# EloDoyard/movie-recommender-system

Hardware: AMD Instinct MI355X
Metric: test-set predictions/sec (kNN k=300, fit+predict+MAE) (higher is better)
Workload: dtype fp16 MFMA similarity filter (fp32 acc) + f64 exact re-rank/prediction

## Files before the change

### movie-recommender-system_amd/csrc/api.cpp

```cpp
#include <math.h>
#include <stdio.h>
#include <string.h>

#include <algorithm>
#include <vector>

#include "engine.h"

using namespace knncf;

namespace knncf {
void launch_first_rows(int64_t n, const int32_t* d_du, const int32_t* d_di, int32_t own_lo, int32_t own_hi,
                       uint32_t* d_first, hipStream_t st);
void launch_length_keys(int32_t count, const int32_t* d_list, const int64_t* d_u_ptr, int32_t max_len, uint64_t* d_key, hipStream_t st);
void launch_collect_new(int32_t U, const uint32_t* d_first, int64_t* d_seq, int64_t epoch, int32_t own_lo, int32_t own_hi,
                        int32_t* d_list, int32_t* d_count, hipStream_t st);
void launch_fallback_keys(int32_t U, const double* d_exact, uint64_t* d_keys, uint32_t* d_vals, hipStream_t st);
void launch_fallback_write(int32_t user, int32_t take, int32_t kcap, const uint32_t* d_sorted_vals,
                           const double* d_exact, int32_t* nbr_idx, double* nbr_sim, int32_t* nbr_cnt,
                           hipStream_t st);
void launch_jaccard_pair(const Train& tr, int32_t u, int32_t v, double* d_out, hipStream_t st);
}

struct StageTimer {
// ... 24 lines not shown
    DArr<bf16_t> Apanel[2];
    DArr<float> S[2];
    DArr<float> S_full;
    DArr<uint32_t> sym_tiles;
    DArr<int32_t> redo_rows;
    int32_t sym_tiles_n = 0;
    hipEvent_t ev_produced[2] = {nullptr, nullptr}, ev_consumed[2] = {nullptr, nullptr}, ev_ready = nullptr;
    int32_t* pinned_cnt = nullptr;
    size_t pinned_cap = 0;
    SelectScratch sel;
    SliceScratch slices;
    NeighborTable pt;
    bool pt_ready = false;
    PersonalRows prow;
    bool prow_ready = false;
    DArr<int32_t> reco_users, reco_items, reco_out_items;
    DArr<double> reco_pred, reco_out_preds;
    DArr<uint8_t> reco_rated;
    QueryScratch query;
    QueryBatchScratch query_batch;
    DArr<int32_t> build_list, build_count;
    DArr<uint32_t> first_row;
    DArr<int32_t> t_du, t_di, t_users, t_items;
    DArr<double> t_pred, t_err, t_ratings, t_partial, scalar_out;
    DArr<unsigned long long> scalar_u64;
    DArr<uint8_t> t_owned;
    DArr<int64_t> t_counts;
    DArr<int32_t> sweep_ks;
    std::vector<uint32_t> h_ukeys, h_ikeys;
    std::vector<int32_t> h_uid;
    knncf_timings tm{};
    std::vector<StageTimer> pending;
    std::vector<hipEvent_t> event_pool;
};

namespace {

hipEvent_t get_event(knncf_handle* h) {
    if (!h->event_pool.empty()) {
        hipEvent_t e = h->event_pool.back();
        h->event_pool.pop_back();
        return e;
    }
    hipEvent_t e;
    KN_HIP(hipEventCreate(&e));
    return e;
// ... 30 lines not shown
template <class F>
int guarded(knncf_handle* h, F&& f) {
    if (!h) return KNNCF_E_INVALID;
    struct DeviceGuard {
        int prev = -1;
        ~DeviceGuard() { if (prev >= 0) (void)hipSetDevice(prev); }
    } guard;
    try {
        int cur = -1;
        if (hipGetDevice(&cur) != hipSuccess) {
            (void)hipGetLastError();
            KN_HIP(hipSetDevice(h->cfg.device));
        } else if (cur != h->cfg.device) {
            guard.prev = cur;
            KN_HIP(hipSetDevice(h->cfg.device));
        }
        f();
        resolve_timers(h);
        return KNNCF_OK;
    } catch (const Error& e) {
        h->err = e.what();
        (void)hipStreamSynchronize(h->stream);
        (void)hipStreamSynchronize(h->stream2);
        (void)hipGetLastError();
        h->pending.clear();
        return e.status;
    } catch (const std::bad_alloc&) {
        h->err = "host allocation failed";
        return KNNCF_E_NOMEM;
    } catch (const std::exception& e) {
        h->err = e.what();
        return KNNCF_E_INVALID;
    }
}

void require_fitted(knncf_handle* h, bool committed = true) {
    KN_REQUIRE(h->fitted, KNNCF_E_STATE, "call knncf_fit first");
    if (committed) KN_REQUIRE(h->committed, KNNCF_E_STATE, "sharded handle: call knncf_shard_commit after the exchange");
}

void load_host_ids(knncf_handle* h) {
    if (!h->h_ukeys.empty() || h->tr.U == 0) return;
    Train& tr = h->tr;
    h->h_ukeys.resize(tr.U);
    h->h_ikeys.resize(tr.I);
    h->h_uid.resize(tr.U);
// ... 86 lines not shown
        const double frac = (double)rows_total / (double)tr.U;
        const double U_pad = (double)round_up(tr.U, 256);
        double best = 1e300;
        H = I;
        for (int64_t cand = 64;; cand += 64) {
            int32_t hc = (int32_t)std::min<int64_t>(cand, I);
            double cost = 2.0 * rows_total * U_pad * (double)round_up(hc, 64) / RATE_DENSE + tail_sq[hc] * frac / RATE_SPARSE;
            if (cost < best) { best = cost; H = hc; }
            if (hc == I) break;
        }
        if (tr.jaccard && (h->cfg.flags & KNNCF_FLAG_F32_PANEL) == 0) H = std::min(H, 2048);
    }
    h->tail_pairs_full = tail_sq[H];
    return H;
}

void build_neighbors(knncf_handle* h, int32_t count) {
    Train& tr = h->tr;
    NeighborTable& nt = h->nt;
    if (count <= 0 || nt.kcap <= 0) return;
    KN_REQUIRE(h->cfg.similarity != KNNCF_SIM_ONE, KNNCF_E_UNSUPPORTED,
               "kNN neighbourhoods with similarityOne: every similarity is 1.0, the neighbourhood is the first k users in Set order — not built");
    hipStream_t st = h->stream;
    if (count > 256) {
        PrepScratch& sc = h->prep;
        sc.k64_a.ensure(count); sc.k64_b.ensure(count); sc.v32_b.ensure(count);
        launch_length_keys(count, h->build_list.p, tr.u_ptr.p, tr.I, sc.k64_a.p, st);
        sort_pairs_u64_u32(sc.sort, sc.k64_a.p, sc.k64_b.p, reinterpret_cast<const uint32_t*>(h->build_list.p), sc.v32_b.p, count, bits_for((uint64_t)tr.I), st);
        KN_HIP(hipMemcpyAsync(h->build_list.p, sc.v32_b.p, (size_t)count * sizeof(int32_t), hipMemcpyDeviceToDevice, st));
    }
    const bool fp16 = (h->cfg.flags & KNNCF_FLAG_BF16_FILTER) == 0;
    const bool s_fp16 = (h->cfg.flags & KNNCF_FLAG_F32_PANEL) == 0;
    h->U_pad = round_up(tr.U, 256);
    const int64_t U_pad = h->U_pad;
    size_t free_b = 0, total_b = 0;
    KN_HIP(hipMemGetInfo(&free_b, &total_b));
    const int64_t s_elem = s_fp16 ? 2 : 4;
    const size_t sym_bytes = (size_t)U_pad * (size_t)U_pad * (size_t)s_elem;
    size_t own = h->S_full.bytes() + h->sel.cand_idx.bytes() + h->sel.cand_approx.bytes() + h->sel.grp_v0.bytes() + h->sel.grp_x.bytes();
    for (int s = 0; s < 2; ++s) own += h->S[s].bytes() + h->Apanel[s].bytes();
    bool use_sym = h->cfg.shard_count == 1 && (int64_t)count * 2 >= tr.U && U_pad / 256 < 65536 &&
                   sym_bytes <= (free_b + own) / 3 && !getenv("KNNCF_DEBUG_NO_SYMMETRIC_GEMM");
    if (use_sym) {
        try {
            h->S_full.ensure((sym_bytes + 3) / 4);
        } catch (const Error& e) {
            if (e.status != KNNCF_E_NOMEM) throw;
            (void)hipGetLastError();
            use_sym = false;
        }
    }
    if (!h->b_ready) {
        h->head = choose_head(h, count, use_sym);
        h->K_pad = round_up(h->head, 64);
        size_t need = (size_t)U_pad * h->K_pad * sizeof(bf16_t);
        KN_REQUIRE(need < free_b + h->Bpanel.bytes(), KNNCF_E_UNSUPPORTED,
                   "dense bf16 user panel does not fit in HBM; lower head_items");
        Stage s(h, &h->tm.densify_ms);
        h->colmap.ensure(tr.I);
        launch_colmap(tr, h->head, h->colmap.p, st);
        h->Bpanel.ensure((size_t)U_pad * h->K_pad);
        launch_densify(tr, nullptr, 0, tr.U, h->colmap.p, h->Bpanel.p, h->K_pad, U_pad, fp16, st);
        if (tr.jaccard) {
            KN_REQUIRE(!s_fp16 || h->head <= 2048, KNNCF_E_UNSUPPORTED, "Jaccard: more than 2048 dense head items need KNNCF_FLAG_F32_PANEL");
            h->row_len.ensure((size_t)row_len_size(tr.U));
            launch_row_len(tr, h->row_len.p, st);
        }
        if (h->head < tr.I) {
            h->te_cnt.ensure(tr.U); h->te_item.ensure(tr.n); h->te_x.ensure(tr.n);
            h->row_tail_abs.ensure(tr.U); h->row_head_sq.ensure(tr.U);
            launch_tail_entries(tr, h->colmap.p, h->te_cnt.p, h->te_item.p, h->te_x.p, h->row_tail_abs.p, h->row_head_sq.p, st);
        }
        h->b_ready = true;
        KN_HIP(hipMemGetInfo(&free_b, &total_b));
    }
    const int64_t K_pad = h->K_pad;
    const int32_t head = h->head;
    h->tm.head_items = head;
    if (use_sym) {
        const int32_t n_tiles = (int32_t)(U_pad / 256);
        if (h->sym_tiles_n != n_tiles) {
            std::vector<uint32_t> list;
            gemm_sym_tile_list(n_tiles, list);
            h->sym_tiles.ensure(list.size());
            KN_HIP(hipMemcpyAsync(h->sym_tiles.p, list.data(), list.size() * sizeof(uint32_t), hipMemcpyHostToDevice, st));
            KN_HIP(hipStreamSynchronize(st));
            h->sym_tiles_n = n_tiles;
        }
        const int64_t n_listed = (int64_t)n_tiles * (n_tiles + 1) / 2;
        Stage s(h, &h->tm.gemm_ms);
        launch_gemm_sym(h->Bpanel.p, h->S_full.p, s_fp16, U_pad, h->K_pad, h->K_pad, U_pad, fp16, !tr.jaccard, h->sym_tiles.p, n_listed, st);
        h->tm.gemm_launches += 1;
        h->tm.gemm_flops_executed += 2.0 * 256.0 * 256.0 * (double)n_listed * (double)h->K_pad;
        h->tm.gemm_flops_algorithmic += 2.0 * (double)count * (double)(tr.U - 1) * (double)h->head;
        KN_HIP(hipMemGetInfo(&free_b, &total_b));
// ... 85 lines not shown
    };
    const bool per_block_redo = !use_sym && n_blocks > 1;
    for (int64_t b = 0; b < n_blocks; ++b) {
        const int64_t rb = b * R;
        const int32_t rows = (int32_t)std::min<int64_t>(R, count - rb);
        const int64_t M = round_up(rows, 256);
        const int32_t* d_rows = h->build_list.p + rb;
        const int slot = (int)(b % slots);
        if (b >= slots) KN_HIP(hipStreamWaitEvent(sp, h->ev_consumed[slot], 0));
        if (!use_sym) {
            Stage s(h, &h->tm.densify_ms, sp);
            launch_densify(tr, d_rows, 0, rows, h->colmap.p, h->Apanel[slot].p, K_pad, M, fp16, sp);
        }
        if (!use_sym) {
            Stage s(h, &h->tm.gemm_ms, sp);
            launch_gemm_nt(h->Apanel[slot].p, h->Bpanel.p, h->S[slot].p, s_fp16, M, U_pad, K_pad, K_pad, K_pad, U_pad, fp16, !tr.jaccard, sp);
            h->tm.gemm_launches += 1;
            h->tm.gemm_flops_executed += 2.0 * (double)M * (double)U_pad * (double)K_pad;
            h->tm.gemm_flops_algorithmic += 2.0 * (double)rows * (double)(tr.U - 1) * (double)head;
        }
        KN_HIP(hipEventRecord(h->ev_produced[slot], sp));
        KN_HIP(hipStreamWaitEvent(sc, h->ev_produced[slot], 0));
        TailEntries te{h->te_cnt.p, h->te_item.p, h->te_x.p, h->row_tail_abs.p, h->row_head_sq.p, h->row_len.p};
        h->prep.join_commit(sc);
        const void* Sblk = use_sym ? (const void*)h->S_full.p : (const void*)h->S[slot].p;
        const int32_t gcap = select_gcap(nt.k);
        auto select_rows = [&](int32_t r0, int32_t nr) {
            Stage s(h, &h->tm.select_ms, sc);
            const void* Sp = use_sym ? Sblk : (const void*)(static_cast<const char*>(Sblk) + (size_t)r0 * (size_t)U_pad * (size_t)s_elem);
            launch_tail_select(tr, h->colmap.p, te, head < tr.I, Sp, use_sym, s_fp16, U_pad, nr, d_rows + r0, nt.k, eps_opnd, eps_rest, cap,
                               h->sel.cand_idx.p + (size_t)r0 * cap, h->sel.cand_approx.p + (size_t)r0 * cap, h->sel.cand_cnt.p + r0, h->sel.cand_eps.p + r0,
                               h->sel.grp_v0.p + (size_t)r0 * gcap, h->sel.grp_x.p + (size_t)r0 * gcap * 8, gcap, sc);
            h->tm.select_launches += 1;
            h->tm.tail_pair_updates += h->tail_pairs_full * ((double)nr / (double)tr.U);
            h->tm.select_row_bytes += (double)s_elem * (double)nr * (double)tr.U;
        };
        const int32_t slices = std::min<int32_t>(8, 8192 / std::max<int32_t>(nt.kcap, 1));
        const char* force_slices = getenv("KNNCF_DEBUG_SLICE_ROWS");
        const int32_t n_heavy = slices < 2                         ? 0
                                : force_slices                     ? std::max<int32_t>(0, std::min<int32_t>(rows, atoi(force_slices)))
                                : (rows >= 4096 && rows <= 65536)  ? std::max<int32_t>(16, rows / 512)
                                                                   : 0;
        select_rows(0, rows);
        if (overlap && !per_block_redo) KN_HIP(hipEventRecord(h->ev_consumed[slot], sc));
        {
            Stage s(h, &h->tm.rerank_ms, sc);
// ... 175 lines not shown
        KN_HIP(hipStreamSynchronize(st));
    }
    const int64_t n_blocks = std::max<int64_t>(1, ceil_div(nu, R));
    for (int64_t b = 0; b < n_blocks; ++b) {
        const int64_t u0 = b * R, u1 = std::min<int64_t>(nu, u0 + R);
        const int64_t r0 = b == 0 ? 0 : first_row[u0], r1 = b + 1 < n_blocks ? first_row[u1] : n;
        if (u1 > u0) {
            Stage s(h, &h->tm.rerank_ms);
            launch_sim_rows(tr, pr, pr.users.p + u0, (int32_t)(u1 - u0), pr.S.p, st);
        }
        Stage s(h, &h->tm.predict_ms);
        launch_fold_rows(tr, pr, r1 - r0, sc.v32_b.p + r0, h->t_du.p, h->t_di.p, d_ratings, pr.slot.p, pr.S.p, d_pred, h->t_err.p,
                         h->t_owned.p, st);
    }
}

void ensure_item_stats(knncf_handle* h) {
    if (h->tr.item_stats_ready) return;
    Stage s(h, &h->tm.prep_ms);
    h->prep.join_commit(h->stream);
    prep_item_stats(h->tr, h->prep, h->stream);
}

int64_t order_test_rows(knncf_handle* h, int64_t n, bool by_item, int32_t cols) {
    Train& tr = h->tr;
    hipStream_t st = h->stream;
    PrepScratch& sc = h->prep;
    sc.k64_a.ensure(n); sc.k64_b.ensure(n); sc.v32_a.ensure(n); sc.v32_b.ensure(n);
    const uint32_t key_limit = (uint32_t)(by_item ? tr.I : tr.U);
    if (h->cfg.shard_count > 1) {
        h->scalar_u64.ensure(1);
        KN_HIP(hipMemsetAsync(h->scalar_u64.p, 0, sizeof(unsigned long long), st));
        KN_HIP(hipMemsetAsync(h->t_err.p, 0, (size_t)cols * (size_t)n * sizeof(double), st));
        KN_HIP(hipMemsetAsync(h->t_owned.p, 0, (size_t)n, st));
        launch_owned_keys(n, by_item ? h->t_di.p : h->t_du.p, h->t_du.p, tr.own_lo, tr.own_hi, h->cfg.shard_rank == 0, key_limit,
                          sc.k64_a.p, sc.v32_a.p, h->scalar_u64.p, st);
        sort_pairs_u64_u32(sc.sort, sc.k64_a.p, sc.k64_b.p, sc.v32_a.p, sc.v32_b.p, n, bits_for((uint64_t)key_limit + 1), st);
        return (int64_t)fetch(h, h->scalar_u64.p, 0);
    }
    launch_user_keys(n, by_item ? h->t_di.p : h->t_du.p, key_limit, sc.k64_a.p, sc.v32_a.p, st);
    sort_pairs_u64_u32(sc.sort, sc.k64_a.p, sc.k64_b.p, sc.v32_a.p, sc.v32_b.p, n, bits_for((uint64_t)key_limit), st);
    return n;
}

void reduce_errors(knncf_handle* h, int64_t n, int32_t cols, double* sums, int64_t* count) {
    hipStream_t st = h->stream;
    const int32_t nb = 1024;
    h->t_partial.ensure((size_t)nb * cols);
    h->t_counts.ensure((size_t)nb * cols);
    for (int32_t c = 0; c < cols; ++c)
        launch_reduce_err(h->t_err.p + (size_t)c * n, h->t_owned.p, n, h->t_partial.p + (size_t)c * nb, h->t_counts.p + (size_t)c * nb, nb, st);
    std::vector<double> hp((size_t)nb * cols);
    std::vector<int64_t> hc((size_t)nb * cols);
    KN_HIP(hipMemcpyAsync(hp.data(), h->t_partial.p, hp.size() * sizeof(double), hipMemcpyDeviceToHost, st));
    KN_HIP(hipMemcpyAsync(hc.data(), h->t_counts.p, hc.size() * sizeof(int64_t), hipMemcpyDeviceToHost, st));
    KN_HIP(hipStreamSynchronize(st));
    for (int32_t c = 0; c < cols; ++c) {
        double s_ = 0.0;
        int64_t c_ = 0;
        for (int32_t b = 0; b < nb; ++b) { s_ += hp[(size_t)c * nb + b]; c_ += hc[(size_t)c * nb + b]; }
        if (sums) sums[c] = s_;
        if (count && c == 0) *count = c_;
    }
}

// ... 9 lines not shown
    KN_REQUIRE(d_users && d_items, KNNCF_E_INVALID, "null test arrays");
    int kind = predictor;
    NeighborTable* table = &h->nt;
    bool stream = false;
    if (predictor == KNNCF_PRED_PERSONALIZED) {
        if (h->cfg.similarity == KNNCF_SIM_ONE) {
            kind = KNNCF_PRED_BASELINE_RDD;
        } else if (personalized_streams(h)) {
            ensure_personal_rows(h);
            stream = true;
        } else {
            ensure_personalized_table(h);
            kind = KNNCF_PRED_KNN;
            table = &h->pt;
        }
    }
    KN_REQUIRE(stream || (kind >= KNNCF_PRED_GLOBAL_AVG && kind <= KNNCF_PRED_KNN), KNNCF_E_INVALID, "unknown predictor");
    if (kind == KNNCF_PRED_ITEM_AVG || kind == KNNCF_PRED_BASELINE || kind == KNNCF_PRED_BASELINE_RDD) ensure_item_stats(h);
    ensure_test_scratch(h, n);
    {
        Stage s(h, &h->tm.predict_ms);
        launch_dense_ids(tr, d_users, d_items, n, h->t_du.p, h->t_di.p, st);
    }
    if (kind == KNNCF_PRED_KNN && table == &h->nt) ensure_neighbors_for_rows(h, n);
    h->prep.join_commit(st);
    double* pred = d_pred_out ? d_pred_out : h->t_pred.p;
    if (stream) predict_personal_rows(h, d_ratings, n, pred);
    {
        Stage s(h, &h->tm.predict_ms);
        const uint32_t* d_order = nullptr;
        const bool by_item = tr.ib_words > 0 && tr.ib_words * 12 <= 48 * 1024;
        int64_t n_rows = n;
        if (kind == KNNCF_PRED_KNN) {
            n_rows = order_test_rows(h, n, by_item, 1);
            d_order = h->prep.v32_b.p;
        }
        if (n_rows > 0 && !stream)
            launch_predict(tr, table, kind, n_rows, h->t_du.p, h->t_di.p, d_ratings, d_order, by_item, pred, h->t_err.p, h->t_owned.p,
                           h->cfg.shard_rank == 0, st);
        if (sum_abs_err || count) reduce_errors(h, n, 1, sum_abs_err, count);
    }
}

void check_sweep_ks(const int32_t* ks, int32_t n_k) {
    KN_REQUIRE(ks && n_k >= 1 && n_k <= 64, KNNCF_E_INVALID, "sweep: 1 .. 64 values of k");
    for (int32_t q = 0; q < n_k; ++q)
        KN_REQUIRE(ks[q] >= 1 && ks[q] <= 2048 && (q == 0 || ks[q] > ks[q - 1]), KNNCF_E_INVALID,
                   "sweep: k must be strictly ascending in [1, 2048]");
}

void run_mae_sweep(knncf_handle* h, const int32_t* ks, int32_t n_k, const int32_t* d_users, const int32_t* d_items,
                   const double* d_ratings, int64_t n, double* sums, int64_t* count, double* d_pred) {
    check_sweep_ks(ks, n_k);
    require_fitted(h);
    KN_REQUIRE(h->cfg.similarity != KNNCF_SIM_ONE, KNNCF_E_UNSUPPORTED,
               "kNN neighbourhoods with similarityOne: every similarity is 1.0, the neighbourhood is the first k users in Set order — not built");
    KN_REQUIRE(n >= 0, KNNCF_E_INVALID, "negative row count");
    for (int32_t q = 0; q < n_k; ++q) sums[q] = 0.0;
    *count = 0;
    if (n == 0) return;
    KN_REQUIRE(d_users && d_items && d_ratings, KNNCF_E_INVALID, "null test arrays");
    Train& tr = h->tr;
    hipStream_t st = h->stream;
    struct Restore {
        knncf_handle* h;
        int32_t k;
        ~Restore() {
            h->cfg.k = k;
            try { reset_neighbors(h); } catch (const Error&) {}
        }
    } restore{h, h->cfg.k};
    h->cfg.k = ks[n_k - 1];
    reset_neighbors(h);
    ensure_test_scratch(h, n);
    h->t_err.ensure((size_t)n_k * n);
    {
        Stage s(h, &h->tm.predict_ms);
        launch_dense_ids(tr, d_users, d_items, n, h->t_du.p, h->t_di.p, st);
    }
    ensure_neighbors_for_rows(h, n);
    h->prep.join_commit(st);
    std::vector<int32_t> hk(ks, ks + n_k);
    h->sweep_ks.ensure(64);
    KN_HIP(hipMemcpyAsync(h->sweep_ks.p, hk.data(), (size_t)n_k * sizeof(int32_t), hipMemcpyHostToDevice, st));
    {
        Stage s(h, &h->tm.predict_ms);
        const int64_t n_rows = order_test_rows(h, n, true, n_k);
        if (n_rows > 0)
            launch_predict_sweep(tr, h->nt, h->sweep_ks.p, n_k, n_rows, n, h->t_du.p, h->t_di.p, d_ratings, h->prep.v32_b.p, d_pred,
                                 h->t_err.p, h->t_owned.p, h->cfg.shard_rank == 0, st);
        reduce_errors(h, n, n_k, sums, count);
    }
}

void do_fit_device(knncf_handle* h, const int32_t* d_users, const int32_t* d_items, const double* d_ratings, int64_t n) {
    KN_REQUIRE(n > 0 && d_users && d_items && d_ratings, KNNCF_E_INVALID, "fit: null or empty input");
    Train& tr = h->tr;
    hipStream_t st = h->stream;
    h->fitted = h->committed = false;
    h->short_rows = -1;
    h->b_ready = false;
    h->pt_ready = false;
    h->prow_ready = false;
    h->h_ukeys.clear(); h->h_ikeys.clear(); h->h_uid.clear();
    tr.n = n;
    tr.jaccard = h->cfg.similarity == KNNCF_SIM_JACCARD;
    {
        Stage s(h, &h->tm.prep_ms);
        if (tr.user_raw.p != d_users) {
            tr.user_raw.alloc(n); tr.item_raw.alloc(n); tr.rating.alloc(n);
            KN_HIP(hipMemcpyAsync(tr.user_raw.p, d_users, n * sizeof(int32_t), hipMemcpyDeviceToDevice, st));
            KN_HIP(hipMemcpyAsync(tr.item_raw.p, d_items, n * sizeof(int32_t), hipMemcpyDeviceToDevice, st));
// ... 401 lines not shown
}

int knncf_create(const knncf_config* cfg, knncf_handle** out) {
    if (!cfg || !out || cfg->struct_size != sizeof(knncf_config)) return KNNCF_E_INVALID;
    if (cfg->shard_count < 1 || cfg->shard_rank < 0 || cfg->shard_rank >= cfg->shard_count || cfg->k < 0)
        return KNNCF_E_INVALID;
    if (cfg->similarity < KNNCF_SIM_COSINE || cfg->similarity > KNNCF_SIM_JACCARD) return KNNCF_E_INVALID;
    int ndev = 0;
    if (hipGetDeviceCount(&ndev) != hipSuccess || ndev <= 0 || cfg->device < 0 || cfg->device >= ndev) {
        (void)hipGetLastError();
        return KNNCF_E_NODEVICE;
    }
    hipDeviceProp_t prop;
    if (hipGetDeviceProperties(&prop, cfg->device) != hipSuccess) return KNNCF_E_NODEVICE;
    if (strncmp(prop.gcnArchName, "gfx950", 6) != 0) return KNNCF_E_NODEVICE;
    knncf_handle* h = new (std::nothrow) knncf_handle();
    if (!h) return KNNCF_E_NOMEM;
    h->cfg = *cfg;
    if (hipSetDevice(cfg->device) != hipSuccess || hipStreamCreateWithFlags(&h->stream, hipStreamNonBlocking) != hipSuccess ||
        hipStreamCreateWithFlags(&h->stream2, hipStreamNonBlocking) != hipSuccess) {
        delete h;
        return KNNCF_E_HIP;
    }
    bool ok = hipEventCreateWithFlags(&h->ev_ready, hipEventDisableTiming) == hipSuccess;
    for (int s = 0; s < 2; ++s) {
        ok = ok && hipEventCreateWithFlags(&h->ev_produced[s], hipEventDisableTiming) == hipSuccess;
        ok = ok && hipEventCreateWithFlags(&h->ev_consumed[s], hipEventDisableTiming) == hipSuccess;
    }
    if (!ok) {
        knncf_destroy(h);
        return KNNCF_E_HIP;
    }
    *out = h;
    return KNNCF_OK;
}

void knncf_destroy(knncf_handle* h) {
    if (!h) return;
    (void)hipSetDevice(h->cfg.device);
    (void)hipStreamSynchronize(h->stream);
    for (auto& t : h->pending) { (void)hipEventDestroy(t.a); (void)hipEventDestroy(t.b); }
    for (auto e : h->event_pool) (void)hipEventDestroy(e);
    if (h->stream2) (void)hipStreamSynchronize(h->stream2);
    if (h->ev_ready) (void)hipEventDestroy(h->ev_ready);
    for (int s = 0; s < 2; ++s) {
        if (h->ev_produced[s]) (void)hipEventDestroy(h->ev_produced[s]);
// ... 446 lines not shown
```

### movie-recommender-system_amd/csrc/engine.h

```cpp
#pragma once

#include <string>
#include <vector>

#include "common.h"

namespace knncf {

typedef __bf16 bf16_t;

inline int32_t select_gcap(int32_t k) { return 8192 * (int32_t)((k + 511) / 512 > 1 ? (k + 511) / 512 : 1); }
static constexpr int SELECT_TCOLS = 16384;
static_assert(SELECT_TCOLS <= 16384 && (SELECT_TCOLS & (SELECT_TCOLS - 1)) == 0, "it_pack: 16-bit cell byte address");

struct SortWorkspace {
    DArr<char> tmp;
    DArr<size_t> count;
};
void sort_pairs_u64_u32(SortWorkspace& ws, const uint64_t* kin, uint64_t* kout, const uint32_t* vin,
                        uint32_t* vout, size_t n, int end_bit, hipStream_t st);
void sort_keys_u32(SortWorkspace& ws, const uint32_t* kin, uint32_t* kout, size_t n, hipStream_t st);
void sort_pairs_u32_u32(SortWorkspace& ws, const uint32_t* kin, uint32_t* kout, const uint32_t* vin, uint32_t* vout, size_t n,
                        int end_bit, hipStream_t st);
size_t unique_u32(SortWorkspace& ws, const uint32_t* sorted_in, uint32_t* out, size_t n, hipStream_t st);
// ... 36 lines not shown
    int64_t own_p0 = 0, own_p1 = 0;
    bool jaccard = false;
};

enum : uint32_t { ST_NONFINITE = 1u, ST_DUPLICATE = 2u, ST_NOT_DYADIC = 4u, ST_LONG_ROW = 16u };

struct PrepScratch {
    SortWorkspace sort;
    DArr<uint64_t> k64_a, k64_b;
    DArr<uint32_t> v32_a, v32_b, k32_a, k32_b;
    DArr<int32_t> du_row, di_row;
    DArr<uint32_t> perm_f;
    DArr<uint32_t> status;
    DArr<int32_t> idrange;
    DArr<uint32_t> ucnt, utile;
    DArr<int32_t> long_rows;
    DArr<double> dsum;
    DArr<uint4> rec;
    hipStream_t aux = nullptr;
    hipEvent_t ev_fork = nullptr, ev_join = nullptr, ev_commit = nullptr;
    bool commit_pending = false;
    DArr<uint32_t> perm_iu;
    void join_commit(hipStream_t st);
    void ensure_aux();
    void release_all();
    PrepScratch() = default;
    PrepScratch(const PrepScratch&) = delete;
    PrepScratch& operator=(const PrepScratch&) = delete;
    ~PrepScratch();
};

void prep_fit(Train& tr, PrepScratch& sc, int32_t shard_rank, int32_t shard_count, hipStream_t st);
void prep_complete_rows(Train& tr, PrepScratch& sc, hipStream_t st);
void prep_commit(Train& tr, PrepScratch& sc, hipStream_t st);
void prep_item_stats(Train& tr, PrepScratch& sc, hipStream_t st);

void launch_dense_ids(const Train& tr, const int32_t* d_users, const int32_t* d_items, int64_t n,
                      int32_t* d_du, int32_t* d_di, hipStream_t st);

void launch_densify(const Train& tr, const int32_t* d_rows, int32_t row_begin, int32_t n_rows,
                    const int32_t* d_colmap, bf16_t* panel, int64_t ld, int64_t panel_rows, bool fp16,
                    hipStream_t st);
void launch_colmap(const Train& tr, int32_t H, int32_t* d_colmap, hipStream_t st);
void launch_gemm_nt(const bf16_t* A, const bf16_t* B, void* C, bool c_fp16, int64_t M, int64_t N, int64_t K,
                    int64_t lda, int64_t ldb, int64_t ldc, bool fp16, bool clamp, hipStream_t st);

// ... 180 lines not shown
```

### movie-recommender-system_amd/csrc/prep.hip

```cpp
#include <math.h>

#include <algorithm>
#include <vector>

#include <stdlib.h>

#include "engine.h"

namespace knncf {

static constexpr int TPB = 256;
static inline int nblocks(int64_t n, int per = TPB) { return (int)std::max<int64_t>(1, ceil_div(n, per)); }

void PrepScratch::ensure_aux() {
    if (aux) return;
    KN_HIP(hipStreamCreateWithFlags(&aux, hipStreamNonBlocking));
    KN_HIP(hipEventCreateWithFlags(&ev_fork, hipEventDisableTiming));
    KN_HIP(hipEventCreateWithFlags(&ev_join, hipEventDisableTiming));
    KN_HIP(hipEventCreateWithFlags(&ev_commit, hipEventDisableTiming));
}
void PrepScratch::join_commit(hipStream_t st) {
    if (!commit_pending) return;
    KN_HIP(hipStreamWaitEvent(st, ev_commit, 0));
    commit_pending = false;
}
PrepScratch::~PrepScratch() {
    if (aux) { (void)hipStreamSynchronize(aux); (void)hipStreamDestroy(aux); }
    if (ev_fork) (void)hipEventDestroy(ev_fork);
    if (ev_join) (void)hipEventDestroy(ev_join);
    if (ev_commit) (void)hipEventDestroy(ev_commit);
}

void PrepScratch::release_all() {
    sort.tmp.release();
    k64_a.release(); k64_b.release(); v32_a.release(); v32_b.release();
    k32_a.release(); k32_b.release(); du_row.release(); di_row.release(); perm_f.release(); rec.release(); long_rows.release(); ucnt.release(); utile.release(); perm_iu.release();
}

__global__ void k_row_keys(int64_t n, const int32_t* __restrict__ users, const int32_t* __restrict__ items,
                           uint32_t* __restrict__ ukey, uint32_t* __restrict__ ikey) {
    int64_t t = (int64_t)blockIdx.x * blockDim.x + threadIdx.x;
    if (t >= n) return;
    ukey[t] = int_trie_key(users[t]);
    ikey[t] = int_trie_key(items[t]);
}

__global__ void __launch_bounds__(TPB) k_id_range(int64_t n, const int32_t* __restrict__ users, const int32_t* __restrict__ items,
                                                  int32_t* __restrict__ idrange) {
    __shared__ int32_t part[4][TPB / 64];
    int32_t u = 0x7fffffff, i = 0x7fffffff, um = (int32_t)0x80000000, im = (int32_t)0x80000000;
    for (int64_t t = (int64_t)blockIdx.x * TPB + threadIdx.x; t < n; t += (int64_t)gridDim.x * TPB) {
        const int32_t a = users[t], b = items[t];
        u = min(u, a); um = max(um, a);
        i = min(i, b); im = max(im, b);
    }
#pragma unroll
    for (int o = 32; o > 0; o >>= 1) {
// ... 542 lines not shown
}

template <bool SQUARE>
static void fold(const int64_t* seg_ptr, int32_t lo, int32_t hi, const uint32_t* perm, const double* src,
                 double* out, hipStream_t st, int32_t spb = TPB) {
    if (hi <= lo) return;
    k_ordered_fold<SQUARE><<<nblocks(hi - lo, spb), TPB, 0, st>>>(seg_ptr, lo, hi, spb, perm, src, out);
    KN_HIP(hipGetLastError());
}

static uint32_t read_status(PrepScratch& sc, hipStream_t st) {
    uint32_t h = 0;
    KN_HIP(hipMemcpyAsync(&h, sc.status.p, sizeof(uint32_t), hipMemcpyDeviceToHost, st));
    KN_HIP(hipStreamSynchronize(st));
    return h;
}

void prep_fit(Train& tr, PrepScratch& sc, int32_t shard_rank, int32_t shard_count, hipStream_t st) {
    const int64_t n = tr.n;
    KN_REQUIRE(n > 0, KNNCF_E_INVALID, "fit: empty training set");
    KN_REQUIRE(n < (int64_t)1 << 29, KNNCF_E_UNSUPPORTED, "fit: more than 2^29-1 ratings (the kernels address the rating arrays with 32-bit byte offsets)");
    if (sc.aux) KN_HIP(hipStreamSynchronize(sc.aux));
    sc.commit_pending = false;
    sc.status.ensure(4);
    KN_HIP(hipMemsetAsync(sc.status.p, 0, 4 * sizeof(uint32_t), st));
    sc.k32_a.ensure(n); sc.k32_b.ensure(n); sc.v32_a.ensure(n); sc.v32_b.ensure(n);
    sc.k64_a.ensure(n); sc.k64_b.ensure(n);

    uint32_t* ukey_row = sc.k32_a.p;
    uint32_t* ikey_row = sc.v32_a.p;
    bool have_row_keys = false;
    sc.idrange.ensure(4);
    {
        const int32_t init[4] = {0x7fffffff, (int32_t)0x80000000, 0x7fffffff, (int32_t)0x80000000};
        KN_HIP(hipMemcpyAsync(sc.idrange.p, init, sizeof(init), hipMemcpyHostToDevice, st));
    }
    k_id_range<<<(unsigned)std::min<int64_t>(1024, ceil_div(n, TPB)), TPB, 0, st>>>(n, tr.user_raw.p, tr.item_raw.p, sc.idrange.p);
    k_check_dyadic<<<nblocks(n), TPB, 0, st>>>(n, tr.rating.p, sc.status.p);
    KN_HIP(hipGetLastError());
    int32_t rg[4];
    uint32_t early_status = 0;
    KN_HIP(hipMemcpyAsync(rg, sc.idrange.p, sizeof(rg), hipMemcpyDeviceToHost, st));
    KN_HIP(hipMemcpyAsync(&early_status, sc.status.p, sizeof(uint32_t), hipMemcpyDeviceToHost, st));
    KN_HIP(hipStreamSynchronize(st));
    const bool dyadic = !(early_status & ST_NOT_DYADIC);
    const int32_t ID_LIMIT = 1 << 24;
    const bool small_ids = rg[0] >= 0 && rg[2] >= 0 && rg[1] < ID_LIMIT && rg[3] < ID_LIMIT && !getenv("KNNCF_DEBUG_NO_ID_TABLES");
    tr.u_table_n = tr.i_table_n = 0;
    size_t U = 0, I = 0;
    if (small_ids) {
        tr.u_table_n = rg[1] + 1;
        tr.i_table_n = rg[3] + 1;
        tr.u_table.ensure(tr.u_table_n);
        tr.i_table.ensure(tr.i_table_n);
        KN_HIP(hipMemsetAsync(tr.u_table.p, 0xff, (size_t)tr.u_table_n * sizeof(int32_t), st));
        KN_HIP(hipMemsetAsync(tr.i_table.p, 0xff, (size_t)tr.i_table_n * sizeof(int32_t), st));
        k_mark_ids<<<nblocks(n), TPB, 0, st>>>(n, tr.user_raw.p, tr.item_raw.p, tr.u_table.p, tr.i_table.p);
        KN_HIP(hipMemsetAsync(sc.status.p + 2, 0, 2 * sizeof(uint32_t), st));
        k_table_keys<<<nblocks(tr.u_table_n), TPB, 0, st>>>(tr.u_table_n, tr.u_table.p, sc.k32_b.p, sc.status.p + 2);
        k_table_keys<<<nblocks(tr.i_table_n), TPB, 0, st>>>(tr.i_table_n, tr.i_table.p, sc.v32_b.p, sc.status.p + 3);
        KN_HIP(hipGetLastError());
        uint32_t cnt[2];
        KN_HIP(hipMemcpyAsync(cnt, sc.status.p + 2, sizeof(cnt), hipMemcpyDeviceToHost, st));
        KN_HIP(hipStreamSynchronize(st));
        U = cnt[0];
        I = cnt[1];
// ... 155 lines not shown
        if (n > 4) {
            k_make_keys<<<nblocks(n), TPB, 0, st>>>(n, 2, sc.du_row.p, sc.di_row.p, tr.user_raw.p, tr.item_raw.p, sc.k64_a.p, 32);
            sort_pairs_u64_u32(sc.sort, sc.k64_a.p, sc.k64_b.p, sc.perm_f.p, tr.perm_uh.p, n, 32 + ubits, st);
        }
    } else if (!seg_sorts && p1 > p0) {
        const int tbits = bits_for((uint64_t)n);
        k_slice_file_keys<<<nblocks(p1 - p0), TPB, 0, st>>>(p0, p1 - p0, lo, tr.s_user.p, tr.s_t.p, tbits, sc.k64_a.p, sc.v32_a.p);
        KN_HIP(hipGetLastError());
        sort_pairs_u64_u32(sc.sort, sc.k64_a.p, sc.k64_b.p, sc.v32_a.p, tr.perm_uf.p + p0, p1 - p0, tbits + bits_for((uint64_t)(hi - lo)), st);
        if (n > 4) {
            k_slice_hash_keys<<<nblocks(p1 - p0), TPB, 0, st>>>(p1 - p0, lo, tr.perm_uf.p + p0, tr.s_user.p, tr.s_t.p, tr.user_raw.p,
                                                               tr.item_raw.p, sc.k64_a.p);
            KN_HIP(hipGetLastError());
            sort_pairs_u64_u32(sc.sort, sc.k64_a.p, sc.k64_b.p, tr.perm_uf.p + p0, tr.perm_uh.p + p0, p1 - p0,
                               32 + bits_for((uint64_t)(hi - lo)), st);
        }
    }
    KN_HIP(hipGetLastError());
    tr.item_stats_ready = false;

    uint32_t status = read_status(sc, st);
    KN_REQUIRE(!(status & ST_DUPLICATE), KNNCF_E_DUPLICATE, "fit: duplicate (user,item) training rows");
    KN_REQUIRE(!(status & ST_LONG_ROW), KNNCF_E_STATE, "fit: a row longer than the segment sorts take reached them");
    sc.dsum.ensure(2);
    KN_HIP(hipMemsetAsync(sc.dsum.p, 0, 2 * sizeof(double), st));
    if (status & ST_NOT_DYADIC) k_sequential_sum<<<1, TPB, 0, st>>>(n, tr.rating.p, sc.dsum.p);
    else k_exact_sum<<<1024, TPB, 0, st>>>(n, tr.rating.p, sc.dsum.p);
    KN_HIP(hipGetLastError());
    double total = 0.0;
    KN_HIP(hipMemcpyAsync(&total, sc.dsum.p, sizeof(double), hipMemcpyDeviceToHost, st));
    KN_HIP(hipStreamSynchronize(st));
    tr.global_avg = total / (double)n;

    tr.user_avg.alloc(U); tr.user_norm.alloc(U);
    if (shard_count > 1) {
        KN_HIP(hipMemsetAsync(tr.user_avg.p, 0, U * sizeof(double), st));
        KN_HIP(hipMemsetAsync(tr.user_norm.p, 0, U * sizeof(double), st));
    }
    if (hi > lo) {
        fold<false>(tr.u_ptr.p, lo, hi, need_uf ? tr.perm_uf.p : nullptr, tr.s_rating.p, tr.user_norm.p, st);
        k_divide_by_count<<<nblocks(hi - lo), TPB, 0, st>>>(tr.u_ptr.p, lo, hi, tr.user_norm.p, tr.user_avg.p);
        k_deviation<<<nblocks(p1 - p0), TPB, 0, st>>>(p0, p1, tr.s_user.p, tr.s_rating.p, tr.user_avg.p, tr.s_dev.p, sc.status.p);
        fold<true>(tr.u_ptr.p, lo, hi, n > 4 ? tr.perm_uh.p : tr.perm_uf.p, tr.s_dev.p, tr.user_norm.p, st);
        k_sqrt<<<nblocks(hi - lo), TPB, 0, st>>>(lo, hi, tr.user_norm.p, tr.user_norm.p);
        k_preprocess<<<nblocks(p1 - p0), TPB, 0, st>>>(p0, p1, tr.s_user.p, tr.s_dev.p, tr.user_norm.p, tr.s_pre.p);
        KN_HIP(hipGetLastError());
    }
    status = read_status(sc, st);
    KN_REQUIRE(!(status & ST_NONFINITE), KNNCF_E_NONFINITE,
               "fit: non-finite normalized deviation (a user's mean is 1 or 5 with a rating beyond it: scale() == 0)");
}

void prep_complete_rows(Train& tr, PrepScratch& sc, hipStream_t st) {
    const int64_t p0 = tr.own_p0, p1 = tr.own_p1, n = tr.n;
// ... 229 lines not shown
```

Measured before the change: 85.86 million.

## Overlap build-list sort, tail entries and test-row ordering on a side stream

```diff
diff --git a/movie-recommender-system_amd/csrc/api.cpp b/movie-recommender-system_amd/csrc/api.cpp
--- a/movie-recommender-system_amd/csrc/api.cpp
+++ b/movie-recommender-system_amd/csrc/api.cpp
@@ -70,6 +70,7 @@
     DArr<int32_t> build_list, build_count;
     DArr<uint32_t> first_row;
     DArr<int32_t> t_du, t_di, t_users, t_items;
+    DArr<uint32_t> t_order;
     DArr<double> t_pred, t_err, t_ratings, t_partial, scalar_out;
     DArr<unsigned long long> scalar_u64;
     DArr<uint8_t> t_owned;
@@ -146,6 +147,7 @@
         h->err = e.what();
         (void)hipStreamSynchronize(h->stream);
         (void)hipStreamSynchronize(h->stream2);
+        h->prep.drain_side();
         (void)hipGetLastError();
         h->pending.clear();
         return e.status;
@@ -278,13 +280,13 @@
     KN_REQUIRE(h->cfg.similarity != KNNCF_SIM_ONE, KNNCF_E_UNSUPPORTED,
                "kNN neighbourhoods with similarityOne: every similarity is 1.0, the neighbourhood is the first k users in Set order — not built");
     hipStream_t st = h->stream;
-    if (count > 256) {
-        PrepScratch& sc = h->prep;
-        sc.k64_a.ensure(count); sc.k64_b.ensure(count); sc.v32_b.ensure(count);
-        launch_length_keys(count, h->build_list.p, tr.u_ptr.p, tr.I, sc.k64_a.p, st);
-        sort_pairs_u64_u32(sc.sort, sc.k64_a.p, sc.k64_b.p, reinterpret_cast<const uint32_t*>(h->build_list.p), sc.v32_b.p, count, bits_for((uint64_t)tr.I), st);
-        KN_HIP(hipMemcpyAsync(h->build_list.p, sc.v32_b.p, (size_t)count * sizeof(int32_t), hipMemcpyDeviceToDevice, st));
-    }
+    auto sort_build_list = [&](hipStream_t s_, SortWorkspace& ws, DArr<uint64_t>& ka, DArr<uint64_t>& kb, DArr<uint32_t>& vb) {
+        if (count <= 256) return;
+        ka.ensure(count); kb.ensure(count); vb.ensure(count);
+        launch_length_keys(count, h->build_list.p, tr.u_ptr.p, tr.I, ka.p, s_);
+        sort_pairs_u64_u32(ws, ka.p, kb.p, reinterpret_cast<const uint32_t*>(h->build_list.p), vb.p, count, bits_for((uint64_t)tr.I), s_);
+        KN_HIP(hipMemcpyAsync(h->build_list.p, vb.p, (size_t)count * sizeof(int32_t), hipMemcpyDeviceToDevice, s_));
+    };
     const bool fp16 = (h->cfg.flags & KNNCF_FLAG_BF16_FILTER) == 0;
     const bool s_fp16 = (h->cfg.flags & KNNCF_FLAG_F32_PANEL) == 0;
     h->U_pad = round_up(tr.U, 256);
@@ -306,6 +308,13 @@
             use_sym = false;
         }
     }
+    if (!use_sym) sort_build_list(st, h->prep.sort, h->prep.k64_a, h->prep.k64_b, h->prep.v32_b);
+    PrepScratch& side = h->prep;
+    if (use_sym && count > 256) {
+        side.fork_side(st);
+        sort_build_list(side.side, side.side_sort, side.side_k64_a, side.side_k64_b, side.side_v32_a);
+        side.mark_side();
+    }
     if (!h->b_ready) {
         h->head = choose_head(h, count, use_sym);
         h->K_pad = round_up(h->head, 64);
@@ -314,19 +323,24 @@
                    "dense bf16 user panel does not fit in HBM; lower head_items");
         Stage s(h, &h->tm.densify_ms);
         h->colmap.ensure(tr.I);
-        launch_colmap(tr, h->head, h->colmap.p, st);
-        h->Bpanel.ensure((size_t)U_pad * h->K_pad);
-        launch_densify(tr, nullptr, 0, tr.U, h->colmap.p, h->Bpanel.p, h->K_pad, U_pad, fp16, st);
         if (tr.jaccard) {
             KN_REQUIRE(!s_fp16 || h->head <= 2048, KNNCF_E_UNSUPPORTED, "Jaccard: more than 2048 dense head items need KNNCF_FLAG_F32_PANEL");
             h->row_len.ensure((size_t)row_len_size(tr.U));
-            launch_row_len(tr, h->row_len.p, st);
         }
         if (h->head < tr.I) {
             h->te_cnt.ensure(tr.U); h->te_item.ensure(tr.n); h->te_x.ensure(tr.n);
             h->row_tail_abs.ensure(tr.U); h->row_head_sq.ensure(tr.U);
-            launch_tail_entries(tr, h->colmap.p, h->te_cnt.p, h->te_item.p, h->te_x.p, h->row_tail_abs.p, h->row_head_sq.p, st);
-        }
+        }
+        launch_colmap(tr, h->head, h->colmap.p, st);
+        if (tr.jaccard || h->head < tr.I) {
+            side.fork_side(st);
+            if (tr.jaccard) launch_row_len(tr, h->row_len.p, side.side);
+            if (h->head < tr.I)
+                launch_tail_entries(tr, h->colmap.p, h->te_cnt.p, h->te_item.p, h->te_x.p, h->row_tail_abs.p, h->row_head_sq.p, side.side);
+            side.mark_side();
+        }
+        h->Bpanel.ensure((size_t)U_pad * h->K_pad);
+        launch_densify(tr, nullptr, 0, tr.U, h->colmap.p, h->Bpanel.p, h->K_pad, U_pad, fp16, st);
         h->b_ready = true;
         KN_HIP(hipMemGetInfo(&free_b, &total_b));
     }
@@ -458,6 +472,7 @@
         KN_HIP(hipEventRecord(h->ev_produced[slot], sp));
         KN_HIP(hipStreamWaitEvent(sc, h->ev_produced[slot], 0));
         TailEntries te{h->te_cnt.p, h->te_item.p, h->te_x.p, h->row_tail_abs.p, h->row_head_sq.p, h->row_len.p};
+        h->prep.join_side(sc);
         h->prep.join_commit(sc);
         const void* Sblk = use_sym ? (const void*)h->S_full.p : (const void*)h->S[slot].p;
         const int32_t gcap = select_gcap(nt.k);
@@ -679,25 +694,33 @@
     prep_item_stats(h->tr, h->prep, h->stream);
 }
 
-int64_t order_test_rows(knncf_handle* h, int64_t n, bool by_item, int32_t cols) {
-    Train& tr = h->tr;
-    hipStream_t st = h->stream;
+void queue_test_order(knncf_handle* h, int64_t n, bool by_item, int32_t cols) {
+    Train& tr = h->tr;
     PrepScratch& sc = h->prep;
-    sc.k64_a.ensure(n); sc.k64_b.ensure(n); sc.v32_a.ensure(n); sc.v32_b.ensure(n);
+    sc.side_k64_a.ensure(n); sc.side_k64_b.ensure(n); sc.side_v32_a.ensure(n); h->t_order.ensure(n);
     const uint32_t key_limit = (uint32_t)(by_item ? tr.I : tr.U);
-    if (h->cfg.shard_count > 1) {
+    const bool sharded = h->cfg.shard_count > 1;
+    if (sharded) {
         h->scalar_u64.ensure(1);
-        KN_HIP(hipMemsetAsync(h->scalar_u64.p, 0, sizeof(unsigned long long), st));
-        KN_HIP(hipMemsetAsync(h->t_err.p, 0, (size_t)cols * (size_t)n * sizeof(double), st));
-        KN_HIP(hipMemsetAsync(h->t_owned.p, 0, (size_t)n, st));
+        KN_HIP(hipMemsetAsync(h->t_err.p, 0, (size_t)cols * (size_t)n * sizeof(double), h->stream));
+        KN_HIP(hipMemsetAsync(h->t_owned.p, 0, (size_t)n, h->stream));
+    }
+    sc.fork_side(h->stream);
+    hipStream_t sx = sc.side;
+    if (sharded) {
+        KN_HIP(hipMemsetAsync(h->scalar_u64.p, 0, sizeof(unsigned long long), sx));
         launch_owned_keys(n, by_item ? h->t_di.p : h->t_du.p, h->t_du.p, tr.own_lo, tr.own_hi, h->cfg.shard_rank == 0, key_limit,
-                          sc.k64_a.p, sc.v32_a.p, h->scalar_u64.p, st);
-        sort_pairs_u64_u32(sc.sort, sc.k64_a.p, sc.k64_b.p, sc.v32_a.p, sc.v32_b.p, n, bits_for((uint64_t)key_limit + 1), st);
-        return (int64_t)fetch(h, h->scalar_u64.p, 0);
-    }
-    launch_user_keys(n, by_item ? h->t_di.p : h->t_du.p, key_limit, sc.k64_a.p, sc.v32_a.p, st);
-    sort_pairs_u64_u32(sc.sort, sc.k64_a.p, sc.k64_b.p, sc.v32_a.p, sc.v32_b.p, n, bits_for((uint64_t)key_limit), st);
-    return n;
+                          sc.side_k64_a.p, sc.side_v32_a.p, h->scalar_u64.p, sx);
+    } else {
+        launch_user_keys(n, by_item ? h->t_di.p : h->t_du.p, key_limit, sc.side_k64_a.p, sc.side_v32_a.p, sx);
+    }
+    sort_pairs_u64_u32(sc.side_sort, sc.side_k64_a.p, sc.side_k64_b.p, sc.side_v32_a.p, h->t_order.p, n,
+                       bits_for((uint64_t)key_limit + (sharded ? 1 : 0)), sx);
+    sc.mark_side();
+}
+int64_t finish_test_order(knncf_handle* h, int64_t n) {
+    h->prep.join_side(h->stream);
+    return h->cfg.shard_count > 1 ? (int64_t)fetch(h, h->scalar_u64.p, 0) : n;
 }
 
 void reduce_errors(knncf_handle* h, int64_t n, int32_t cols, double* sums, int64_t* count) {
@@ -753,6 +776,8 @@
         Stage s(h, &h->tm.predict_ms);
         launch_dense_ids(tr, d_users, d_items, n, h->t_du.p, h->t_di.p, st);
     }
+    const bool by_item = tr.ib_words > 0 && tr.ib_words * 12 <= 48 * 1024;
+    if (kind == KNNCF_PRED_KNN) queue_test_order(h, n, by_item, 1);
     if (kind == KNNCF_PRED_KNN && table == &h->nt) ensure_neighbors_for_rows(h, n);
     h->prep.join_commit(st);
     double* pred = d_pred_out ? d_pred_out : h->t_pred.p;
@@ -760,11 +785,10 @@
     {
         Stage s(h, &h->tm.predict_ms);
         const uint32_t* d_order = nullptr;
-        const bool by_item = tr.ib_words > 0 && tr.ib_words * 12 <= 48 * 1024;
         int64_t n_rows = n;
         if (kind == KNNCF_PRED_KNN) {
-            n_rows = order_test_rows(h, n, by_item, 1);
-            d_order = h->prep.v32_b.p;
+            n_rows = finish_test_order(h, n);
+            d_order = h->t_order.p;
         }
         if (n_rows > 0 && !stream)
             launch_predict(tr, table, kind, n_rows, h->t_du.p, h->t_di.p, d_ratings, d_order, by_item, pred, h->t_err.p, h->t_owned.p,
@@ -809,6 +833,7 @@
         Stage s(h, &h->tm.predict_ms);
         launch_dense_ids(tr, d_users, d_items, n, h->t_du.p, h->t_di.p, st);
     }
+    queue_test_order(h, n, true, n_k);
     ensure_neighbors_for_rows(h, n);
     h->prep.join_commit(st);
     std::vector<int32_t> hk(ks, ks + n_k);
@@ -816,9 +841,9 @@
     KN_HIP(hipMemcpyAsync(h->sweep_ks.p, hk.data(), (size_t)n_k * sizeof(int32_t), hipMemcpyHostToDevice, st));
     {
         Stage s(h, &h->tm.predict_ms);
-        const int64_t n_rows = order_test_rows(h, n, true, n_k);
+        const int64_t n_rows = finish_test_order(h, n);
         if (n_rows > 0)
-            launch_predict_sweep(tr, h->nt, h->sweep_ks.p, n_k, n_rows, n, h->t_du.p, h->t_di.p, d_ratings, h->prep.v32_b.p, d_pred,
+            launch_predict_sweep(tr, h->nt, h->sweep_ks.p, n_k, n_rows, n, h->t_du.p, h->t_di.p, d_ratings, h->t_order.p, d_pred,
                                  h->t_err.p, h->t_owned.p, h->cfg.shard_rank == 0, st);
         reduce_errors(h, n, n_k, sums, count);
     }
@@ -1266,6 +1291,7 @@
         delete h;
         return KNNCF_E_HIP;
     }
+    h->prep.side = h->stream2;
     bool ok = hipEventCreateWithFlags(&h->ev_ready, hipEventDisableTiming) == hipSuccess;
     for (int s = 0; s < 2; ++s) {
         ok = ok && hipEventCreateWithFlags(&h->ev_produced[s], hipEventDisableTiming) == hipSuccess;
diff --git a/movie-recommender-system_amd/csrc/engine.h b/movie-recommender-system_amd/csrc/engine.h
--- a/movie-recommender-system_amd/csrc/engine.h
+++ b/movie-recommender-system_amd/csrc/engine.h
@@ -82,6 +82,16 @@
     bool commit_pending = false;
     DArr<uint32_t> perm_iu;
     void join_commit(hipStream_t st);
+    hipStream_t side = nullptr;
+    SortWorkspace side_sort;
+    DArr<uint64_t> side_k64_a, side_k64_b;
+    DArr<uint32_t> side_v32_a;
+    hipEvent_t ev_side = nullptr;
+    bool side_pending = false;
+    void fork_side(hipStream_t st);
+    void mark_side();
+    void join_side(hipStream_t st);
+    void drain_side();
     void ensure_aux();
     void release_all();
     PrepScratch() = default;
diff --git a/movie-recommender-system_amd/csrc/prep.hip b/movie-recommender-system_amd/csrc/prep.hip
--- a/movie-recommender-system_amd/csrc/prep.hip
+++ b/movie-recommender-system_amd/csrc/prep.hip
@@ -18,21 +18,43 @@
     KN_HIP(hipEventCreateWithFlags(&ev_fork, hipEventDisableTiming));
     KN_HIP(hipEventCreateWithFlags(&ev_join, hipEventDisableTiming));
     KN_HIP(hipEventCreateWithFlags(&ev_commit, hipEventDisableTiming));
+    KN_HIP(hipEventCreateWithFlags(&ev_side, hipEventDisableTiming));
 }
 void PrepScratch::join_commit(hipStream_t st) {
     if (!commit_pending) return;
     KN_HIP(hipStreamWaitEvent(st, ev_commit, 0));
     commit_pending = false;
+}
+void PrepScratch::fork_side(hipStream_t st) {
+    ensure_aux();
+    KN_HIP(hipEventRecord(ev_fork, st));
+    KN_HIP(hipStreamWaitEvent(side, ev_fork, 0));
+}
+void PrepScratch::mark_side() {
+    KN_HIP(hipEventRecord(ev_side, side));
+    side_pending = true;
+}
+void PrepScratch::join_side(hipStream_t st) {
+    if (!side_pending) return;
+    KN_HIP(hipStreamWaitEvent(st, ev_side, 0));
+    side_pending = false;
+}
+void PrepScratch::drain_side() {
+    if (side) (void)hipStreamSynchronize(side);
+    if (aux) (void)hipStreamSynchronize(aux);
+    side_pending = false;
 }
 PrepScratch::~PrepScratch() {
     if (aux) { (void)hipStreamSynchronize(aux); (void)hipStreamDestroy(aux); }
     if (ev_fork) (void)hipEventDestroy(ev_fork);
     if (ev_join) (void)hipEventDestroy(ev_join);
     if (ev_commit) (void)hipEventDestroy(ev_commit);
+    if (ev_side) (void)hipEventDestroy(ev_side);
 }
 
 void PrepScratch::release_all() {
     sort.tmp.release();
+    side_sort.tmp.release(); side_k64_a.release(); side_k64_b.release(); side_v32_a.release();
     k64_a.release(); k64_b.release(); v32_a.release(); v32_b.release();
     k32_a.release(); k32_b.release(); du_row.release(); di_row.release(); perm_f.release(); rec.release(); long_rows.release(); ucnt.release(); utile.release(); perm_iu.release();
 }
@@ -621,6 +643,7 @@
     KN_REQUIRE(n < (int64_t)1 << 29, KNNCF_E_UNSUPPORTED, "fit: more than 2^29-1 ratings (the kernels address the rating arrays with 32-bit byte offsets)");
     if (sc.aux) KN_HIP(hipStreamSynchronize(sc.aux));
     sc.commit_pending = false;
+    sc.side_pending = false;
     sc.status.ensure(4);
     KN_HIP(hipMemsetAsync(sc.status.p, 0, 4 * sizeof(uint32_t), st));
     sc.k32_a.ensure(n); sc.k32_b.ensure(n); sc.v32_a.ensure(n); sc.v32_b.ensure(n);
@@ -636,11 +659,16 @@
     }
     k_id_range<<<(unsigned)std::min<int64_t>(1024, ceil_div(n, TPB)), TPB, 0, st>>>(n, tr.user_raw.p, tr.item_raw.p, sc.idrange.p);
     k_check_dyadic<<<nblocks(n), TPB, 0, st>>>(n, tr.rating.p, sc.status.p);
+    sc.dsum.ensure(2);
+    KN_HIP(hipMemsetAsync(sc.dsum.p, 0, 2 * sizeof(double), st));
+    k_exact_sum<<<1024, TPB, 0, st>>>(n, tr.rating.p, sc.dsum.p);
     KN_HIP(hipGetLastError());
     int32_t rg[4];
     uint32_t early_status = 0;
+    double total = 0.0;
     KN_HIP(hipMemcpyAsync(rg, sc.idrange.p, sizeof(rg), hipMemcpyDeviceToHost, st));
     KN_HIP(hipMemcpyAsync(&early_status, sc.status.p, sizeof(uint32_t), hipMemcpyDeviceToHost, st));
+    KN_HIP(hipMemcpyAsync(&total, sc.dsum.p, sizeof(double), hipMemcpyDeviceToHost, st));
     KN_HIP(hipStreamSynchronize(st));
     const bool dyadic = !(early_status & ST_NOT_DYADIC);
     const int32_t ID_LIMIT = 1 << 24;
@@ -842,14 +870,13 @@
     uint32_t status = read_status(sc, st);
     KN_REQUIRE(!(status & ST_DUPLICATE), KNNCF_E_DUPLICATE, "fit: duplicate (user,item) training rows");
     KN_REQUIRE(!(status & ST_LONG_ROW), KNNCF_E_STATE, "fit: a row longer than the segment sorts take reached them");
-    sc.dsum.ensure(2);
-    KN_HIP(hipMemsetAsync(sc.dsum.p, 0, 2 * sizeof(double), st));
-    if (status & ST_NOT_DYADIC) k_sequential_sum<<<1, TPB, 0, st>>>(n, tr.rating.p, sc.dsum.p);
-    else k_exact_sum<<<1024, TPB, 0, st>>>(n, tr.rating.p, sc.dsum.p);
-    KN_HIP(hipGetLastError());
-    double total = 0.0;
-    KN_HIP(hipMemcpyAsync(&total, sc.dsum.p, sizeof(double), hipMemcpyDeviceToHost, st));
-    KN_HIP(hipStreamSynchronize(st));
+    if (status & ST_NOT_DYADIC) {
+        KN_HIP(hipMemsetAsync(sc.dsum.p, 0, 2 * sizeof(double), st));
+        k_sequential_sum<<<1, TPB, 0, st>>>(n, tr.rating.p, sc.dsum.p);
+        KN_HIP(hipGetLastError());
+        KN_HIP(hipMemcpyAsync(&total, sc.dsum.p, sizeof(double), hipMemcpyDeviceToHost, st));
+        KN_HIP(hipStreamSynchronize(st));
+    }
     tr.global_avg = total / (double)n;
 
     tr.user_avg.alloc(U); tr.user_norm.alloc(U);
```

New measurement: 85.97 million, median of 6. No clear change (+0.1%).
